# nextpyp/spr_pick

Measured on AMD Instinct MI355X. Metric: train_patches_per_sec, higher is better.
Workload: dtype f32; 1 GPU; BASELINE configs[1]: ssdn --noise_style gaussian --noise_value var, joint mode, 64x64 patches from 4 synthetic 1024x1024 micrographs, batch 32 per GPU, alpha 0.75, tau 0.01, Adam; fp32 MFMA convolutions (Winograd F(2x2,3x3) for the wide 3x3 layers); per_gpu_batch=32, global_batch=32, patch=64, parallelism=single GPU

## Files before the change

include/sprk.h:

```cpp
#ifndef SPRK_H
#define SPRK_H

#include <stddef.h>
#include <stdint.h>

#ifdef __cplusplus
extern "C" {
#endif

#define SPRK_OK 0
#define SPRK_EINVAL (-1)
#define SPRK_EWORKSPACE (-2)
#define SPRK_ELAUNCH (-3)

#define SPRK_ACT_NONE 0
#define SPRK_ACT_LEAKY 1
#define SPRK_ACT_RELU 2

typedef struct sprk_conv_geom {
    int32_t N, C1, C2, Hin, Win, up1;
    int32_t Cout, Hout, Wout;
    int32_t KH, KW, stride, dil, pad_top, pad_left;
    int32_t dtype;
} sprk_conv_geom;

#define SPRK_DT_F32 0
#define SPRK_DT_BF16 1
#define SPRK_DT_F16 2
#define SPRK_DT_MASK 0xff
#define SPRK_DT_FORCE 0x100
#define SPRK_DT_NAIVE 0x200
#define SPRK_DT_PIN 0x400
#define SPRK_DT_X16 0x8000
#define SPRK_DT_Y16 0x10000
#define SPRK_IO2(a, b) ((a) | ((b) << 4))
#define SPRK_IO3(a, b, c) ((a) | ((b) << 4) | ((c) << 8))

typedef struct sprk_conv_epilogue {
    const float *bias, *scale, *shift, *res;
    int32_t res_h, res_w, res_off;
    int32_t act;
    int32_t up2;
} sprk_conv_epilogue;

#define SPRK_ABI_VERSION 430
const char *sprk_last_error(void);
int sprk_version(void);
size_t sprk_struct_bytes(int which);
long sprk_launch_count(void);
long sprk_wino_launch_count(void);
long sprk_mask1x1_launch_count(void);
long sprk_gemm1x1_launch_count(void);
void sprk_gemm1x1_enable(int on);
long sprk_wgrad1x1_launch_count(void);
void sprk_wgrad1x1_enable(int on);
long sprk_conv16_launch_count(void);
long sprk_wgrad16_launch_count(void);

size_t sprk_conv2d_fwd_ws_bytes(const sprk_conv_geom *g);
int sprk_conv2d_fwd(const float *x, const float *x2, const float *w, float *y,
                    const sprk_conv_geom *g, const sprk_conv_epilogue *ep,
                    void *ws, size_t ws_bytes, void *stream);
size_t sprk_conv2d_bwd_data_ws_bytes(const sprk_conv_geom *g);
int sprk_conv2d_bwd_data(const float *gy, const float *w, float *gin, const sprk_conv_geom *g,
                         void *ws, size_t ws_bytes, void *stream);
size_t sprk_head1x1_fwd_ws_bytes(int K0, int N1);
int sprk_head1x1_fwd(const float *f, const float *w1, const float *b1, const float *w2, const float *b2,
                     const float *w3, const float *b3, float *out, int B, int K0, int N1, int N3, long HW, void *ws,
                     size_t ws_bytes, void *stream);

int sprk_head1x1_unrot_fwd(const float *d, const float *w1, const float *b1, const float *w2, const float *b2,
                           const float *w3, const float *b3, float *out, int B, int C, int P, int N3, void *ws,
                           size_t ws_bytes, void *stream);

int sprk_conv2d_bwd_data_masked(const float *gy, const float *w, float *gin, const sprk_conv_geom *g,
                                const float *mask_y, int mask_act, void *ws, size_t ws_bytes, void *stream);
int sprk_conv2d_bwd_data_mask_fused(const sprk_conv_geom *g);
int sprk_conv2d_storage16(const sprk_conv_geom *g, const sprk_conv_epilogue *ep);
size_t sprk_conv2d_bwd_weight_ws_bytes(const sprk_conv_geom *g);
int sprk_conv2d_bwd_weight(const float *x, const float *x2, const float *gy, float *gw,
                           const sprk_conv_geom *g, void *ws, size_t ws_bytes, void *stream);
#define SPRK_VARIANT_INTS 24
#define SPRK_STAGE_NONE (-2)
#define SPRK_STAGE_REFUSED (-1)
#define SPRK_STAGE_DIRECT 0
#define SPRK_STAGE_STEM 1
#define SPRK_STAGE_16BIT 2
#define SPRK_STAGE_WINOGRAD 3
#define SPRK_STAGE_MASK1X1 4
#define SPRK_STAGE_MFMA 5
#define SPRK_STAGE_GEMM1X1 6
#define SPRK_STAGE_WGRAD1X1 7
int sprk_conv2d_variant(int which, const sprk_conv_geom *g, const sprk_conv_epilogue *ep, const void *x, const void *x2,
                        const void *y_or_gy, int32_t *out);
int sprk_conv2d_last_variant(int which, int32_t *out);

#define SPRK_DT_WPREP 0x800
#define SPRK_DT_WPREP_KIND(kind) (((kind) & 7) << 12)
#define SPRK_DT_WPREP_KIND_OF(dtype) (((dtype) >> 12) & 7)
typedef struct sprk_wprep_item {
    const float *w;
    void *dst;
    int32_t kind, blocks;
    int32_t p[12];
} sprk_wprep_item;
int sprk_conv2d_fwd_wprep(const float *w, const sprk_conv_geom *g, const sprk_conv_epilogue *ep, void *ws,
                          size_t ws_bytes, sprk_wprep_item *item);
int sprk_conv2d_bwd_data_wprep(const float *w, const sprk_conv_geom *g, void *ws, size_t ws_bytes, sprk_wprep_item *item);
int sprk_prepare_weights(const sprk_wprep_item *items, int n, void *stream);

size_t sprk_act_bwd_ws_bytes(int N, int C, int HW);
int sprk_act_bwd(const void *gy, const void *y, void *gpre, float *gbias, int act,
                 int N, int C, int H, int W, int up2, long g_image_stride, int io,
                 void *ws, size_t ws_bytes, void *stream);
#define SPRK_RED_NONE 0
#define SPRK_RED_ROWS 1
#define SPRK_RED_COLS 2
#define SPRK_RED_WGRAD 3
typedef struct sprk_reduce_item {
    const float *src;
    float *dst;
    int kind, parts, n, K, Cout, CoutP;
} sprk_reduce_item;
int sprk_conv2d_bwd_weight_partial(const float *x, const float *x2, const float *gy, float *gw,
                                   const sprk_conv_geom *g, void *ws, size_t ws_bytes,
                                   sprk_reduce_item *item, void *stream);
int sprk_act_bwd_partial(const void *gy, const void *y, void *gpre, float *gbias, int act,
                         int N, int C, int H, int W, int up2, long g_image_stride, int io,
                         void *ws, size_t ws_bytes, sprk_reduce_item *item, void *stream);
int sprk_reduce_items(const sprk_reduce_item *items, int n, void *stream);

int sprk_concat_up_bwd(const float *gin, float *ga, float *gb, int N, int C1, int C2, int H, int W,
                       int up1, void *stream);

int sprk_shift_maxpool2_fwd(const void *x, void *y, int NC, int H, int W, int shift, int io, void *stream);
int sprk_shift_maxpool2_bwd(const void *gy, const void *x, void *gx, int NC, int H, int W, int shift, int act,
                            int io, void *stream);
int sprk_rot4_stack_fwd(const float *x, float *y, int B, int C, int P, void *stream);
int sprk_rot4_stack_bwd(const float *gy, float *gx, int B, int C, int P, void *stream);
int sprk_unrot4_shift_concat_fwd(const void *d, void *f, int B, int C, int P, int io, void *stream);
int sprk_unrot4_shift_concat_bwd(const void *gf, void *gd, int B, int C, int P, int io, void *stream);
int sprk_unrot_act_bwd_eligible(int B, int C, int P, int act);
int sprk_conv2d_fwd_unrot_eligible(const sprk_conv_geom *g, const sprk_conv_epilogue *ep);
int sprk_conv2d_fwd_unrot(const float *x, const float *x2, const float *w, float *f, const sprk_conv_geom *g,
                          const sprk_conv_epilogue *ep, void *ws, size_t ws_bytes, void *stream);
// ... 120 lines not shown
```

spr_pick_amd/_lib.py:

```python
import ctypes
import os

_HERE = os.path.dirname(os.path.abspath(__file__))
LIB_PATH = os.environ.get("SPRK_LIB") or os.path.join(_HERE, "libsprk.so")

ACT_NONE, ACT_LEAKY, ACT_RELU = 0, 1, 2
DT_F32, DT_BF16, DT_F16 = 0, 1, 2
DT_NAIVE = 0x200
DT_WPREP = 0x800
DT_X16, DT_Y16 = 0x8000, 0x10000
DT_PIN = 0x400
DT_FORCE = 0x100
DTYPES = {"f32": DT_F32, "fp32": DT_F32, "bf16": DT_BF16, "f16": DT_F16, "fp16": DT_F16,
          "bf16!": DT_BF16 | DT_FORCE, "f16!": DT_F16 | DT_FORCE}

c_f = ctypes.c_void_p
c_i = ctypes.c_int
c_vp = ctypes.c_void_p
c_sz = ctypes.c_size_t


class ConvGeom(ctypes.Structure):
    _fields_ = [(n, ctypes.c_int32) for n in
                ("N", "C1", "C2", "Hin", "Win", "up1", "Cout", "Hout", "Wout",
                 "KH", "KW", "stride", "dil", "pad_top", "pad_left", "dtype")]


class ConvEpilogue(ctypes.Structure):
    _fields_ = [("bias", c_vp), ("scale", c_vp), ("shift", c_vp), ("res", c_vp),
                ("res_h", ctypes.c_int32), ("res_w", ctypes.c_int32), ("res_off", ctypes.c_int32),
                ("act", ctypes.c_int32), ("up2", ctypes.c_int32)]


class AdamItem(ctypes.Structure):
    _fields_ = [("p", c_vp), ("g", c_vp), ("m", c_vp), ("v", c_vp), ("n", ctypes.c_long)]


class ReduceItem(ctypes.Structure):
    _fields_ = [("src", c_vp), ("dst", c_vp), ("kind", ctypes.c_int32), ("parts", ctypes.c_int32), ("n", ctypes.c_int32),
                ("K", ctypes.c_int32), ("Cout", ctypes.c_int32), ("CoutP", ctypes.c_int32)]


class WprepItem(ctypes.Structure):
    _fields_ = [("w", c_vp), ("dst", c_vp), ("kind", ctypes.c_int32), ("blocks", ctypes.c_int32), ("p", ctypes.c_int32 * 12)]


_SIGS = {
    "sprk_last_error": (ctypes.c_char_p, []),
    "sprk_version": (c_i, []),
    "sprk_struct_bytes": (c_sz, [c_i]),
    "sprk_launch_count": (ctypes.c_long, []),
    "sprk_wino_launch_count": (ctypes.c_long, []),
    "sprk_mask1x1_launch_count": (ctypes.c_long, []),
    "sprk_gemm1x1_launch_count": (ctypes.c_long, []),
    "sprk_gemm1x1_enable": (None, [c_i]),
    "sprk_wgrad1x1_launch_count": (ctypes.c_long, []),
    "sprk_wgrad1x1_enable": (None, [c_i]),
    "sprk_conv16_launch_count": (ctypes.c_long, []),
    "sprk_wgrad16_launch_count": (ctypes.c_long, []),
    "sprk_conv2d_fwd_ws_bytes": (c_sz, [ctypes.POINTER(ConvGeom)]),
    "sprk_conv2d_fwd": (c_i, [c_f, c_f, c_f, c_f, ctypes.POINTER(ConvGeom), ctypes.POINTER(ConvEpilogue), c_vp, c_sz, c_vp]),
    "sprk_conv2d_fwd_wprep": (c_i, [c_f, ctypes.POINTER(ConvGeom), ctypes.POINTER(ConvEpilogue), c_vp, c_sz, ctypes.POINTER(WprepItem)]),
    "sprk_conv2d_bwd_data_wprep": (c_i, [c_f, ctypes.POINTER(ConvGeom), c_vp, c_sz, ctypes.POINTER(WprepItem)]),
    "sprk_prepare_weights": (c_i, [ctypes.POINTER(WprepItem), c_i, c_vp]),
    "sprk_head1x1_fwd_ws_bytes": (c_sz, [c_i, c_i]),
    "sprk_head1x1_fwd": (c_i, [c_f, c_f, c_f, c_f, c_f, c_f, c_f, c_f, c_i, c_i, c_i, c_i, ctypes.c_long, c_vp, c_sz, c_vp]),
    "sprk_head1x1_unrot_fwd": (c_i, [c_f, c_f, c_f, c_f, c_f, c_f, c_f, c_f, c_i, c_i, c_i, c_i, c_vp, c_sz, c_vp]),
    "sprk_conv2d_bwd_data_ws_bytes": (c_sz, [ctypes.POINTER(ConvGeom)]),
    "sprk_conv2d_bwd_data": (c_i, [c_f, c_f, c_f, ctypes.POINTER(ConvGeom), c_vp, c_sz, c_vp]),
    "sprk_conv2d_bwd_data_masked": (c_i, [c_f, c_f, c_f, ctypes.POINTER(ConvGeom), c_f, c_i, c_vp, c_sz, c_vp]),
    "sprk_conv2d_bwd_weight_ws_bytes": (c_sz, [ctypes.POINTER(ConvGeom)]),
    "sprk_conv2d_storage16": (c_i, [ctypes.POINTER(ConvGeom), ctypes.POINTER(ConvEpilogue)]),
    "sprk_conv2d_bwd_weight": (c_i, [c_f, c_f, c_f, c_f, ctypes.POINTER(ConvGeom), c_vp, c_sz, c_vp]),
    "sprk_conv2d_bwd_weight_partial": (c_i, [c_f, c_f, c_f, c_f, ctypes.POINTER(ConvGeom), c_vp, c_sz, ctypes.POINTER(ReduceItem), c_vp]),
    "sprk_act_bwd_partial": (c_i, [c_f, c_f, c_f, c_f, c_i, c_i, c_i, c_i, c_i, c_i, ctypes.c_long, c_i, c_vp, c_sz, ctypes.POINTER(ReduceItem), c_vp]),
    "sprk_reduce_items": (c_i, [ctypes.POINTER(ReduceItem), c_i, c_vp]),
    "sprk_act_bwd_ws_bytes": (c_sz, [c_i, c_i, c_i]),
    "sprk_act_bwd": (c_i, [c_f, c_f, c_f, c_f, c_i, c_i, c_i, c_i, c_i, c_i, ctypes.c_long, c_i, c_vp, c_sz, c_vp]),
    "sprk_concat_up_bwd": (c_i, [c_f, c_f, c_f, c_i, c_i, c_i, c_i, c_i, c_i, c_vp]),
    "sprk_shift_maxpool2_fwd": (c_i, [c_f, c_f, c_i, c_i, c_i, c_i, c_i, c_vp]),
    "sprk_shift_maxpool2_bwd": (c_i, [c_f, c_f, c_f, c_i, c_i, c_i, c_i, c_i, c_i, c_vp]),
    "sprk_rot4_stack_fwd": (c_i, [c_f, c_f, c_i, c_i, c_i, c_vp]),
    "sprk_rot4_stack_bwd": (c_i, [c_f, c_f, c_i, c_i, c_i, c_vp]),
    "sprk_unrot4_shift_concat_fwd": (c_i, [c_f, c_f, c_i, c_i, c_i, c_i, c_vp]),
    "sprk_unrot4_shift_concat_bwd": (c_i, [c_f, c_f, c_i, c_i, c_i, c_i, c_vp]),
    "sprk_unrot_act_bwd_eligible": (c_i, [c_i, c_i, c_i, c_i]),
    "sprk_conv2d_fwd_unrot_eligible": (c_i, [ctypes.POINTER(ConvGeom), ctypes.POINTER(ConvEpilogue)]),
    "sprk_conv2d_bwd_data_mask_fused": (c_i, [ctypes.POINTER(ConvGeom)]),
    "sprk_conv2d_variant": (c_i, [c_i, ctypes.POINTER(ConvGeom), ctypes.POINTER(ConvEpilogue), c_vp, c_vp, c_vp,
                                  ctypes.POINTER(ctypes.c_int32)]),
    "sprk_conv2d_last_variant": (c_i, [c_i, ctypes.POINTER(ctypes.c_int32)]),
    "sprk_conv2d_fwd_unrot": (c_i, [c_f, c_f, c_f, c_f, ctypes.POINTER(ConvGeom), ctypes.POINTER(ConvEpilogue), c_vp, c_sz, c_vp]),
    "sprk_unrot_act_bwd": (c_i, [c_f, c_f, c_f, c_f, c_i, c_i, c_i, c_i, c_vp, c_sz, ctypes.POINTER(ReduceItem), c_vp]),
    "sprk_bn_ws_bytes": (c_sz, [c_i, c_i, c_i, c_i]),
    "sprk_bn_train_fwd": (c_i, [c_f, c_f, c_f, c_f, c_f, c_f, c_f, c_f, c_i, c_i, c_i, c_i, ctypes.c_float, ctypes.c_float, c_i, c_vp, c_sz, c_vp]),
    "sprk_bn_eval_fwd": (c_i, [c_f, c_f, c_f, c_f, c_f, c_f, c_i, c_i, c_i, ctypes.c_float, c_i, c_vp]),
    "sprk_bn_train_bwd": (c_i, [c_f, c_f, c_f, c_f, c_f, c_f, c_f, c_f, c_f, c_i, c_i, c_i, c_i, c_i, c_vp, c_sz, c_vp]),
    "sprk_crop_add_fwd": (c_i, [c_f, c_f, c_f, ctypes.c_long, c_i, c_i, c_i, c_i, c_i, c_i, c_vp]),
    "sprk_crop_embed_bwd": (c_i, [c_f, c_f, ctypes.c_long, c_i, c_i, c_i, c_i, c_i, c_i, c_vp]),
    "sprk_noise_std_fwd": (c_i, [c_f, c_f, c_f, c_i, c_i, c_vp]),
    "sprk_noise_std_bwd": (c_i, [c_f, c_f, c_f, c_i, c_i, c_vp]),
    "sprk_joint_loss_fwd": (c_i, [c_f, c_f, c_f, c_f, c_f, c_f, c_i, c_i, c_i, c_i, ctypes.c_float, ctypes.c_float, c_vp]),
    "sprk_joint_loss_bwd": (c_i, [c_f, c_f, c_f, c_f, c_f, c_f, c_f, c_i, c_i, c_i, c_i, ctypes.c_float, ctypes.c_float, c_vp]),
    "sprk_reparam_fwd": (c_i, [c_f, c_f, c_f, c_i, c_i, c_vp]),
    "sprk_reparam_bwd": (c_i, [c_f, c_f, c_f, c_f, c_i, c_i, c_vp]),
    "sprk_adam_multi": (c_i, [c_vp, c_vp, c_i, c_i, c_f, c_f, c_f, ctypes.c_float, ctypes.c_float, ctypes.c_float, c_vp]),
    "sprk_adam_multi_skip": (c_i, [c_vp, c_vp, c_i, c_i, c_f, c_f, c_f, ctypes.c_float, ctypes.c_float, ctypes.c_float, c_vp, c_vp]),
    "sprk_unscale_check": (c_i, [c_f, ctypes.c_long, c_f, c_vp, c_vp]),
    "sprk_loss_scale_update": (c_i, [c_f, c_f, c_vp, c_vp, c_vp, c_vp, ctypes.c_float, ctypes.c_float, c_i, c_vp]),
    "sprk_pu_loss": (c_i, [c_f, c_f, c_f, c_i, ctypes.c_float, c_f, c_f, c_vp]),
# ... 70 lines not shown
```

spr_pick_amd/csrc/conv.hip:

```cpp
#include "common.h"
#include "conv16.h"
#include "gemm1x1.h"
#include "mask1x1.h"
#include "wgrad16.h"
#include "wgrad1x1.h"
#include "wino.h"
#include "wprep_dev.h"

#include <cstdlib>

#include "conv_dev.h"
#include "io_dev.h"


namespace {

inline bool naive_of(const sprk_conv_geom *g) { return (g->dtype & SPRK_DT_NAIVE) != 0; }

constexpr int kZeroFloats = 256;
__device__ __attribute__((aligned(64))) float g_zero_block[kZeroFloats];

__device__ __forceinline__ void stage_planes(float *dst, const float *base, long imgStride, long cs, int nch, int N,
                                             int Hin, int Win, int Ws, int up, int vec, const float *zeros,
                                             const PlaneGeom &g, int n0, int iy0, int ixa, int lw, int lane) {
    const int imgElems = g.inRows * g.pitch;
    const int planeElems = g.NI * imgElems;
    const int per = vec ? 256 : 64;
    const int nGroups = (planeElems + per - 1) / per;
    const int nw = g.nw;
    const int gstart = g.deal ? 0 : lw, gstep = g.deal ? 1 : nw, cstep = g.deal ? nw : 1;
    for (int gi = gstart; gi < nGroups; gi += gstep) {
        const int e = vec ? gi * 256 + lane * 4 : gi * 64 + lane;
        const int il = fast_div(e, g.invImg);
        const int rem = e - il * imgElems;
        const int r = fast_div(rem, g.invPitch);
        const int j = rem - r * g.pitch;
        const int n = n0 + il, iy = iy0 + r, ix = ixa + j;
        const bool inb = e < planeElems;
        const bool ok = inb && n < N && (unsigned)iy < (unsigned)Hin && (unsigned)ix < (unsigned)Win;
        const int cl0 = g.deal ? (lw + nw - (gi % nw)) % nw : 0;
        const float *p = base + (long)n * imgStride + (up ? (long)(iy >> 1) * Ws + (ix >> 1) : (long)iy * Ws + ix) +
                         (long)cl0 * cs;
        long step = (long)cstep * cs;
        if (!ok) {
            p = zeros + lane * 4;
            step = 0;
        }
        float *d = dst + gi * per + cl0 * g.cplane;
        for (int cl = cl0; cl < nch; cl += cstep) {
            if (inb) {
                if (vec)
                    dma16(p, d);
                else
                    dma4(p, d);
            }
            p += step;
            d += cstep * g.cplane;
        }
// ... 1622 lines not shown
    return rc == sprk::kWprepDescribed ? (int)SPRK_OK : rc;
}

int sprk_conv2d_bwd_data(const float *gy, const float *w, float *gin, const sprk_conv_geom *g, void *ws,
                         size_t ws_bytes, void *stream) {
    return sprk_conv2d_bwd_data_masked(gy, w, gin, g, nullptr, SPRK_ACT_NONE, ws, ws_bytes, stream);
}

int sprk_conv2d_bwd_data_masked(const float *gy, const float *w, float *gin, const sprk_conv_geom *g,
                                const float *mask_y, int mask_act, void *ws, size_t ws_bytes, void *stream) {
    sprk::WprepScope scope(nullptr, g ? g->dtype : 0);
    return scope.verify(conv_dispatch(true, gy, nullptr, w, gin, g, nullptr, mask_y, mask_act, ws, ws_bytes, stream));
}

int sprk_conv2d_bwd_data_mask_fused(const sprk_conv_geom *g) {
    if (!g || check_geom(g) != SPRK_OK || naive_of(g) || g->stride != 1 || g->up1) return 0;
    const sprk::Corr c(*g);
    if (c.dt() != SPRK_DT_F32 && sprk::conv16_eligible(c)) return 0;
    if (c.dtype & (SPRK_DT_X16 | SPRK_DT_Y16)) return 0;
    if (sprk::wino_eligible(c)) return 1;
    FwdPlan p;
    return (plan_fwd(c, &p) && mask1x1_takes(g, c, p)) ? 1 : 0;
}

int sprk_conv2d_bwd_data_wprep(const float *w, const sprk_conv_geom *g, void *ws, size_t ws_bytes, sprk_wprep_item *item) {
    SPRK_REQUIRE(item && w && ws, "conv2d_bwd_data_wprep: null argument");
    *item = sprk_wprep_item{};
    sprk::WprepScope scope(item, 0);
    const int rc = conv_dispatch(true, (const float *)ws, nullptr, w, (float *)ws, g, nullptr, nullptr, SPRK_ACT_NONE, ws,
                                 ws_bytes, nullptr);
    return rc == sprk::kWprepDescribed ? (int)SPRK_OK : rc;
}

static size_t wgrad_ws_bytes(const sprk_conv_geom &g) {
    size_t need = sprk::wgrad16_ws_bytes(g);
    WgPlan p;
    if (sprk::wino_wgrad_eligible(g)) need = std::max(need, sprk::wino_wgrad_ws_bytes(g));
    if (plan_wgrad(&g, &p)) need = std::max(need, p.wsBytes);
    return need;
}

size_t sprk_conv2d_bwd_weight_ws_bytes(const sprk_conv_geom *g) { return g ? wgrad_ws_bytes(*g) : 0; }

static bool wgrad1x1_takes(const sprk_conv_geom *g, const WgPlan &p, const WgVariant &v) {
    const int W = g->Wout, H = g->Hout;
    const bool rows64 = W % 64 == 0 || ((W == 4 || W == 8 || W == 16 || W == 32) && H % (64 / W) == 0 && H * W >= 64);
    return sprk::g_wgrad1x1_on.load(std::memory_order_relaxed) && (g->dtype & SPRK_DT_MASK) == SPRK_DT_F32 &&
           !(g->dtype & (SPRK_DT_X16 | SPRK_DT_Y16)) && !naive_of(g) && g->KH == 1 && g->KW == 1 && g->stride == 1 &&
           g->pad_top == 0 && g->pad_left == 0 && g->C2 == 0 && !g->up1 && g->Hin == g->Hout && g->Win == g->Wout &&
           v.stage == SPRK_STAGE_MFMA && p.xrow && v.MODE == 1 && p.IT == 3 && p.NT == 6 && p.CKW <= sprk::kWgrad1x1Rows &&
           rows64 && (long)sprk::kWgrad1x1Rows * H * W * 4 < (1L << 31);
}

static WgVariant wg_route(const sprk_conv_geom *g, const void *x, const void *x2, const void *gy, WgPlan *p) {
    WgVariant v{};
    const bool naive = naive_of(g);
    if (!naive && sprk::wgrad16_ws_bytes(*g)) {
        v.stage = SPRK_STAGE_16BIT;
        sprk::wgrad16_variant(*g, v.rec16);
    } else if (g->dtype & (SPRK_DT_X16 | SPRK_DT_Y16)) {
        v.stage = SPRK_STAGE_REFUSED;
    } else if (!naive && sprk::wino_wgrad_eligible(*g)) {
        v.stage = SPRK_STAGE_WINOGRAD;
        v.wino = sprk::wino_wgrad_variant(*g);
    } else if (naive || !plan_wgrad(g, p)) {
        v.stage = SPRK_STAGE_DIRECT;
    } else {
        bool refused;
        v = wg_variant(g, *p, x, x2, gy, &refused);
        v.stage = refused ? SPRK_STAGE_REFUSED : SPRK_STAGE_MFMA;
        if (wgrad1x1_takes(g, *p, v)) v.stage = SPRK_STAGE_WGRAD1X1;
    }
    return v;
}

static int wgrad_dispatch(const float *x, const float *x2, const float *gy, float *gw, const sprk_conv_geom *g, void *ws,
                          size_t ws_bytes, sprk_reduce_item *item, void *stream) {
    const char *who = "conv2d_bwd_weight";
    if (item) *item = sprk_reduce_item{nullptr, nullptr, SPRK_RED_NONE, 0, 0, 0, 0, 0};
    if (int rc = check_geom(g)) return rc;
    SPRK_REQUIRE(x && gy && gw, "conv2d_bwd_weight: null tensor");
    SPRK_REQUIRE(g->C2 == 0 || x2, "conv2d_bwd_weight: C2 > 0 but x2 is null");
    hipStream_t s = (hipStream_t)stream;

    WgPlan p;
    const WgVariant v = wg_route(g, x, x2, gy, &p);
    t_last_wg = v;

    if (v.stage == SPRK_STAGE_16BIT) {
        if (int rc = sprk::check_ws(who, ws, ws_bytes, sprk::wgrad16_ws_bytes(*g))) return rc;
        return sprk::wgrad16_run(*g, x, x2, gy, gw, ws, item, s);
    }
    if (int rc = check_storage32(who, g->dtype)) return rc;

    if (v.stage == SPRK_STAGE_WINOGRAD) {
        if (int rc = sprk::check_ws(who, ws, ws_bytes, sprk::wino_wgrad_ws_bytes(*g))) return rc;
        return sprk::wino_wgrad(*g, v.wino, x, x2, gy, gw, ws, item, s);
    }

    if (v.stage == SPRK_STAGE_DIRECT) {
        DirectArgs a{x, x2, nullptr, gy, gw, *g, sprk::kNoEpilogue};
        hipLaunchKernelGGL(conv_bwd_weight_direct_kernel, dim3(g->Cout * (g->C1 + g->C2)), dim3(256), 0, s, a);
        return sprk::check_launch("conv_bwd_weight_direct");
    }
    if (int rc = sprk::check_ws(who, ws, ws_bytes, p.wsBytes)) return rc;
    SPRK_REQUIRE(v.stage != SPRK_STAGE_REFUSED,
                 "conv2d_bwd_weight: 1x1 row staging needs 16-byte aligned x / gy and < 2^28-element tiles");
    float *wsf = (float *)ws;
    if (v.stage == SPRK_STAGE_WGRAD1X1) {
        const sprk::Wgrad1x1Call c{x, gy, wsf + kZeroFloats, g->N, g->C1, g->Cout, p.CoutP, g->Hout * g->Wout,
                                   p.nTiles, p.tilesPerGroup, p.groups, p.CKW, p.nChunks, p.nblkN};
        sprk::prof_begin(1, sprk::conv_flops(*g), s);
        if (int rc = sprk::wgrad1x1_run(c, s)) return rc;
        sprk::prof_end(1, s);
        if (int rc2 = sprk::check_launch("wgrad1x1")) return rc2;
    } else {
        WgArgs a;
        if (int rc = wgrad_args(g, p, v, x, x2, gy, wsf, a)) return rc;
        sprk::prof_begin(1, sprk::conv_flops(*g), s);
        if (int rc = launch_wg(a, p, v, s)) return rc;
        sprk::prof_end(1, s);
        if (int rc2 = sprk::check_launch("conv_wgrad_mfma")) return rc2;
    }
    const int K = (g->C1 + g->C2) * g->KH * g->KW;
    const sprk_reduce_item it{wsf + kZeroFloats, gw, SPRK_RED_WGRAD, p.groups, 0, K, g->Cout, p.CoutP};
    return sprk::finish_or_defer(it, item, s);
}

static void variant_out(const FwdVariant &v, int32_t *out) {
    if (v.stage == SPRK_STAGE_16BIT) {
        out[0] = v.stage;
        for (int i = 1; i < SPRK_VARIANT_INTS; ++i) out[i] = v.rec16[i];
        return;
    }
    if (v.stage == SPRK_STAGE_WINOGRAD) {
        const sprk::WinoVariant &w = v.wino;
        const int f[] = {v.stage, w.NT, w.SQ, w.UNROT, w.groups, w.lastCh, w.nc1, w.nch, w.r1, w.r2, w.pairs, w.sw, w.gridX,
                         w.ntiles, w.tpwMin, w.tpwMax, w.xcd, w.tilesX, w.tilesY, w.padT, w.padL, w.mode};
        static_assert(sizeof(f) / sizeof(f[0]) <= SPRK_VARIANT_INTS, "the record fits");
        for (int i = 0; i < SPRK_VARIANT_INTS; ++i) out[i] = i < (int)(sizeof(f) / sizeof(f[0])) ? f[i] : 0;
        return;
    }
    const int f[] = {v.stage, v.MT, v.NT, v.RB, v.XTAB, v.small, v.stages, v.ragged_k, v.latency, v.vec1, v.vec2, v.vec4,
                     v.colOff, v.up1, v.c2, v.taps, v.CK, v.nChunks, v.blocks};
    for (int i = 0; i < SPRK_VARIANT_INTS; ++i) out[i] = i < (int)(sizeof(f) / sizeof(f[0])) ? f[i] : 0;
}
static void variant_out(const WgVariant &v, int32_t *out) {
    if (v.stage == SPRK_STAGE_16BIT) {
        out[0] = v.stage;
        for (int i = 1; i < SPRK_VARIANT_INTS; ++i) out[i] = v.rec16[i];
        return;
    }
    if (v.stage == SPRK_STAGE_WINOGRAD) {
        const sprk::WinoWgVariant &w = v.wino;
        int f[SPRK_VARIANT_INTS] = {v.stage, w.launches};
        for (int i = 0; i < w.launches; ++i) f[2 + 3 * i] = w.l[i].MT, f[3 + 3 * i] = w.l[i].ch, f[4 + 3 * i] = w.l[i].parts;
        int srcMask = 0;
        for (int i = 0; i < w.launches; ++i) srcMask |= w.l[i].src << i;
        const int t[] = {w.regionsX, w.regionsY, w.cx, w.cy, w.padT, w.padL, w.Cout, w.xcdMask, srcMask};
        static_assert(14 + sizeof(t) / sizeof(t[0]) <= SPRK_VARIANT_INTS, "the record fits");
        for (int i = 0; i < (int)(sizeof(t) / sizeof(t[0])); ++i) f[14 + i] = t[i];
        for (int i = 0; i < SPRK_VARIANT_INTS; ++i) out[i] = f[i];
        return;
    }
    const int f[] = {v.stage, v.IT, v.NT, v.WJ, v.MODE, v.xrow, v.xtab, v.g4, v.vec1, v.vec2, v.chunks, v.groups, v.up1, v.c2,
                     v.tiles};
    for (int i = 0; i < SPRK_VARIANT_INTS; ++i) out[i] = i < (int)(sizeof(f) / sizeof(f[0])) ? f[i] : 0;
}
// ... 128 lines not shown
```

spr_pick_amd/csrc/core.hip:

```cpp
#include "common.h"
#include "wprep_dev.h"
#include "conv16.h"
#include "gemm1x1.h"
#include "wgrad1x1.h"
#include "wgrad16.h"

#include <mutex>
#include <tuple>
#include <vector>

namespace sprk {

static thread_local char t_error[512] = "";
std::atomic<long> g_launches{0}, g_wino_launches{0}, g_mask1x1_launches{0};

void set_error(const char *fmt, ...) {
    va_list ap;
    va_start(ap, fmt);
    vsnprintf(t_error, sizeof(t_error), fmt, ap);
    va_end(ap);
}

constexpr int kMaxDev = 64;
int num_cus() {
    static std::atomic<int> cus[kMaxDev];
    int dev = 0;
    if (hipGetDevice(&dev) != hipSuccess || dev < 0 || dev >= kMaxDev) return 256;
    int v = cus[dev].load(std::memory_order_relaxed);
    if (v == 0) {
        if (hipDeviceGetAttribute(&v, hipDeviceAttributeMultiprocessorCount, dev) != hipSuccess || v <= 0) v = 256;
        cus[dev].store(v, std::memory_order_relaxed);
    }
    return v;
}

int lds_optin(const void *kernel, size_t bytes, const char *what) {
    if (bytes <= 64 * 1024) return SPRK_OK;
    static std::mutex mu;
    static std::vector<std::tuple<int, const void *, size_t>> done;
    int dev = 0;
    (void)hipGetDevice(&dev);
    std::lock_guard<std::mutex> lk(mu);
    for (auto &d : done)
        if (std::get<0>(d) == dev && std::get<1>(d) == kernel && std::get<2>(d) >= bytes) return SPRK_OK;
    if (hipFuncSetAttribute(kernel, hipFuncAttributeMaxDynamicSharedMemorySize, (int)bytes) != hipSuccess) {
        set_error("%s: cannot reserve %zu bytes of LDS", what, bytes);
        return SPRK_ELAUNCH;
    }
    done.emplace_back(dev, kernel, bytes);
    return SPRK_OK;
}

struct ProfRec {
    hipEvent_t a, b;
    int kclass;
    double flops, bytes;
};
// ... 187 lines not shown
    set_error("prepared weights: the workspace holds a transform of another kind than this call's kernel path reads");
    return SPRK_EINVAL;
}
bool wprep_describing() { return t_wprep_describe != nullptr; }
int wprep_site(const sprk_wprep_item &it, hipStream_t s) {
    if (t_wprep_describe) {
        *t_wprep_describe = it;
        return kWprepDescribed;
    }
    if (t_wprep_skip) {
        t_wprep_seen = it.kind;
        if (t_wprep_expect && it.kind != t_wprep_expect) {
            set_error("prepared weights: the workspace holds a transform of another kind than this call's kernel path reads");
            return SPRK_EINVAL;
        }
        return SPRK_OK;
    }
    return wprep_launch(&it, 1, s);
}

}

extern "C" {

int sprk_prepare_weights(const sprk_wprep_item *items, int n, void *stream) {
    SPRK_REQUIRE(n >= 0 && (n == 0 || items), "prepare_weights: bad arguments");
    return sprk::wprep_launch(items, n, (hipStream_t)stream);
}

int sprk_reduce_items(const sprk_reduce_item *items, int n, void *stream) {
    SPRK_REQUIRE(n >= 0 && (n == 0 || items), "reduce_items: bad arguments");
    return sprk::reduce_items(items, n, (hipStream_t)stream);
}

const char *sprk_last_error(void) { return sprk::t_error; }
int sprk_version(void) { return SPRK_ABI_VERSION; }
size_t sprk_struct_bytes(int which) {
    switch (which) {
    case 0: return sizeof(sprk_conv_geom);
    case 1: return sizeof(sprk_conv_epilogue);
    case 2: return sizeof(sprk_reduce_item);
    case 3: return sizeof(sprk_adam_item);
    case 4: return sizeof(sprk_wprep_item);
    default: return 0;
    }
}
long sprk_launch_count(void) { return sprk::g_launches.load(); }
long sprk_wino_launch_count(void) { return sprk::g_wino_launches.load(); }
long sprk_mask1x1_launch_count(void) { return sprk::g_mask1x1_launches.load(); }
long sprk_gemm1x1_launch_count(void) { return sprk::g_gemm1x1_launches.load(); }
void sprk_gemm1x1_enable(int on) { sprk::g_gemm1x1_on.store(on ? 1 : 0); }
long sprk_wgrad1x1_launch_count(void) { return sprk::g_wgrad1x1_launches.load(); }
void sprk_wgrad1x1_enable(int on) { sprk::g_wgrad1x1_on.store(on ? 1 : 0); }
long sprk_conv16_launch_count(void) { return sprk::conv16_launches() + sprk::wgrad16_launches(); }
long sprk_wgrad16_launch_count(void) { return sprk::wgrad16_launches(); }

void sprk_prof_enable(int on) {
    std::lock_guard<std::mutex> lk(sprk::g_prof_mu);
    sprk::g_prof_mask = on;
}

int sprk_prof_collect(int kclass, long *launches, double *ms, double *flops) {
    return sprk_prof_collect_bytes(kclass, launches, ms, flops, nullptr);
}

int sprk_prof_collect_bytes(int kclass, long *launches, double *ms, double *flops, double *bytes) {
    std::lock_guard<std::mutex> lk(sprk::g_prof_mu);
    long n = 0;
    double t = 0.0, f = 0.0, by = 0.0;
    std::vector<sprk::ProfRec> keep;
    for (auto &r : sprk::g_recs) {
        if (r.kclass != kclass) {
            keep.push_back(r);
            continue;
        }
        float dt = 0.f;
        if (hipEventSynchronize(r.b) == hipSuccess && hipEventElapsedTime(&dt, r.a, r.b) == hipSuccess) {
            ++n;
            t += dt;
            f += r.flops;
            by += r.bytes;
        }
        sprk::g_pool.push_back({r.a, r.b});
    }
    sprk::g_recs.swap(keep);
    if (launches) *launches = n;
    if (ms) *ms = t;
    if (flops) *flops = f;
    if (bytes) *bytes = by;
    return SPRK_OK;
}

}
```

Measured before the change: 2034 patches/s.

## Add specialized MFMA weight-gradient kernel for 3x3 fp32 convolutions

Adds a dedicated wgrad3x3 kernel for stride-1 3x3 fp32 weight-gradient convolutions that the generic MFMA path would otherwise handle. It stages 48-channel input chunks and output-gradient tiles into double-buffered LDS with buffer DMA, then feeds 16x16x4 MFMAs from shared LDS images across the 27 k-tiles of a chunk. It is enabled by default and gated on a narrow set of plan parameters. The aim is more data reuse and overlap of loads with compute in the wide 3x3 layers' weight gradients, at the cost of large LDS use and a hand-scheduled pipeline that is more fragile. Scratch benchmarking scripts are included.

```diff
diff --git a/include/sprk.h b/include/sprk.h
--- a/include/sprk.h
+++ b/include/sprk.h
@@ -54,6 +54,8 @@
 void sprk_gemm1x1_enable(int on);
 long sprk_wgrad1x1_launch_count(void);
 void sprk_wgrad1x1_enable(int on);
+long sprk_wgrad3x3_launch_count(void);
+void sprk_wgrad3x3_enable(int on);
 long sprk_conv16_launch_count(void);
 long sprk_wgrad16_launch_count(void);
 
@@ -91,6 +93,7 @@
 #define SPRK_STAGE_MFMA 5
 #define SPRK_STAGE_GEMM1X1 6
 #define SPRK_STAGE_WGRAD1X1 7
+#define SPRK_STAGE_WGRAD3X3 8
 int sprk_conv2d_variant(int which, const sprk_conv_geom *g, const sprk_conv_epilogue *ep, const void *x, const void *x2,
                         const void *y_or_gy, int32_t *out);
 int sprk_conv2d_last_variant(int which, int32_t *out);
diff --git a/scratch/wgrad3x3_bench.py b/scratch/wgrad3x3_bench.py
--- /dev/null
+++ b/scratch/wgrad3x3_bench.py
@@ -0,0 +1,110 @@
+import ctypes
+import json
+import statistics
+import sys
+
+import torch
+
+from spr_pick_amd import _lib, ops
+
+GEOM = ("N", "C1", "C2", "Hin", "Win", "up1", "Cout", "Hout", "Wout", "KH", "KW", "stride", "dil", "pad_top", "pad_left", "dtype")
+
+
+def last_record(L):
+    out = (ctypes.c_int32 * 24)()
+    L.sprk_conv2d_last_variant(2, out)
+    return list(out)
+
+
+def do_list(path):
+    sys.path.insert(0, ".")
+    from bench import make_cfg
+    from spr_pick_amd import Denoiser, graph_step, synthetic
+    L = _lib.lib()
+    calls = []
+
+    def wrap(name, igeom):
+        real = getattr(L, name)
+
+        def f(*a):
+            rc = real(*a)
+            g = a[igeom]._obj
+            calls.append({"geom": [int(getattr(g, k)) for k in GEOM],
+                          "aligned16": [(ctypes.cast(p, ctypes.c_void_p).value or 0) % 16 == 0 for p in a[:3]],
+                          "record": last_record(L)})
+            return rc
+        setattr(L, name, f)
+
+    wrap("sprk_conv2d_bwd_weight", 4)
+    wrap("sprk_conv2d_bwd_weight_partial", 4)
+    dev = torch.device("cuda:0")
+    torch.manual_seed(0)
+    den = Denoiser(make_cfg(), device=dev, mode="joint")
+    den.train()
+    st = graph_step.GraphedTrainStep(den, 32, 64, 0.75, 0.01, graph=False)
+    inp, tgt = synthetic.patch_batches(1, 32, [synthetic.micrograph(i) for i in range(2)], seed=100, device=dev)[0]
+    st(inp, tgt, eager=True)
+    torch.cuda.synchronize()
+    calls.clear()
+    st(inp, tgt, eager=True)
+    torch.cuda.synchronize()
+    json.dump({"geom_fields": GEOM, "calls": calls}, open(path, "w"), indent=0)
+    for i, c in enumerate(calls):
+        g, r = dict(zip(GEOM, c["geom"])), c["record"]
+        print("%3d N%4d C%3d+%3d %3dx%-3d up%d -> %3d k%d s%d d%d pad %d,%d  stage %d IT %d NT %d WJ %d MODE %d chunks %d groups %d c2 %d tiles %d" % (
+            i, g["N"], g["C1"], g["C2"], g["Hin"], g["Win"], g["up1"], g["Cout"], g["KH"], g["stride"], g["dil"], g["pad_top"],
+            g["pad_left"], r[0], r[1], r[2], r[3], r[4], r[10], r[11], r[13], r[14]))
+
+
+def do_run(path, reps, only):
+    L, S, dev = _lib.lib(), torch.ops.sprk, torch.device("cuda:0")
+    have = "sprk_wgrad3x3_enable" in _lib.EXPORTS
+    calls = [c for c in json.load(open(path))["calls"]
+             if c["record"][0] == 5 and c["record"][4] == 2 and c["geom"][9] == 3 and c["geom"][10] == 3]
+    seen, uniq = set(), []
+    for c in calls:
+        if tuple(c["geom"]) not in seen:
+            seen.add(tuple(c["geom"]))
+            uniq.append(c)
+    gen = torch.Generator().manual_seed(1)
+    for i, c in enumerate(uniq):
+        if only and i not in only:
+            continue
+        g = dict(zip(GEOM, c["geom"]))
+        x = torch.randn(g["N"], g["C1"], g["Hin"], g["Win"], generator=gen).to(dev)
+        x2 = torch.randn(g["N"], g["C2"], g["Hin"], g["Win"], generator=gen).to(dev) if g["C2"] else None
+        gy = torch.randn(g["N"], g["Cout"], g["Hout"], g["Wout"], generator=gen).to(dev)
+        gw = torch.empty(g["Cout"], g["C1"] + g["C2"], 3, 3, device=dev)
+        geom = [g[k] for k in GEOM]
+        res = {}
+        for on in ((0, 1) if have else (None,)):
+            if on is not None:
+                L.sprk_wgrad3x3_enable(on)
+            ts = []
+            for _ in range(reps):
+                a, b = torch.cuda.Event(enable_timing=True), torch.cuda.Event(enable_timing=True)
+                a.record()
+                S.conv2d_bwd_weight(x, x2, gy, geom, gw, False)
+                b.record()
+                torch.cuda.synchronize()
+                ts.append(a.elapsed_time(b) * 1e3)
+            res[on] = gw.clone()
+            r = last_record(L)
+            print("CALL %d switch %s N %d C %d+%d %dx%d -> %d pad %d,%d  stage %d IT %d NT %d chunks %d groups %d tiles %d  "
+                  "median %.1f us min %.1f (reduction included; %.1f TF)" % (
+                      i, on, g["N"], g["C1"], g["C2"], g["Hin"], g["Win"], g["Cout"], g["pad_top"], g["pad_left"], r[0], r[1],
+                      r[2], r[10], r[11], r[14], statistics.median(ts), min(ts),
+                      18.0 * g["N"] * g["Hout"] * g["Wout"] * (g["C1"] + g["C2"]) * g["Cout"] / statistics.median(ts) * 1e-6),
+                  flush=True)
+        if have:
+            print("    on == off: %s" % torch.equal(res[0].view(torch.int32), res[1].view(torch.int32)), flush=True)
+        del x, x2, gy, gw, res
+        torch.cuda.empty_cache()
+
+
+if __name__ == "__main__":
+    if sys.argv[1] == "list":
+        do_list(sys.argv[2])
+    else:
+        do_run(sys.argv[2], int(sys.argv[3]) if len(sys.argv) > 3 else 5,
+               [int(t) for t in sys.argv[4].split(",")] if len(sys.argv) > 4 else [])
diff --git a/scratch/wgrad3x3_step_trace.py b/scratch/wgrad3x3_step_trace.py
--- /dev/null
+++ b/scratch/wgrad3x3_step_trace.py
@@ -0,0 +1,39 @@
+import csv
+import glob
+import os
+import re
+import sys
+
+d, steps = sys.argv[1], int(sys.argv[2]) if len(sys.argv) > 2 else 8
+pat = re.compile("conv_wgrad_mfma_kernel|wgrad1x1_kernel|wgrad3x3_kernel")
+DRIFT = (("gemm1x1_kernel<2", None), ("wgrad1x1_kernel", None), ("wino_conv_kernel<6, 0, 1", None),
+         ("unrot_act_bwd64_kernel", None), ("wino_wgrad_kernel<3", "131072"))
+
+
+def short(n):
+    n = re.sub(r"\(anonymous namespace\)::", "", n)
+    n = re.sub(r"^void ", "", n)
+    return n.split("(")[0][:48]
+
+
+def med(v):
+    v = sorted(v)
+    return v[len(v) // 2]
+
+
+for f in sorted(glob.glob(os.path.join(d, "**", "*kernel_trace.csv"), recursive=True)):
+    rows = sorted((int(r["Start_Timestamp"]), short(r["Kernel_Name"]), r.get("Grid_Size_X", ""),
+                   (int(r["End_Timestamp"]) - int(r["Start_Timestamp"])) / 1e3) for r in csv.DictReader(open(f)))
+    main = [r for r in rows if pat.search(r[1])]
+    gs = [r[2] for r in main]
+    period = next(m for m in range(1, len(gs) // 3) if gs[-m:] == gs[-2 * m:-m] == gs[-3 * m:-2 * m] and len(set(gs[-m:])) > 1)
+    use = min(steps, len(gs) // period - 1)
+    tail = main[-use * period:]
+    print("%s: %d launches, period %d, %d steps used" % (os.path.basename(f), len(main), period, use))
+    for p in range(period):
+        v = [tail[s * period + p][3] for s in range(use)]
+        print("POS %2d %-44s grid %7s  median %.1f us  min %.1f" % (p, tail[p][1], tail[p][2], med(v), min(v)))
+    for name, grid in DRIFT:
+        v = [r[3] for r in rows if name in r[1] and (grid is None or r[2] == grid)]
+        if v:
+            print("DRIFT %-44s grid %7s  n %d  median %.1f us" % (name, grid or "any", len(v), med(v)))
diff --git a/scratch/wgrad3x3_summary.py b/scratch/wgrad3x3_summary.py
--- /dev/null
+++ b/scratch/wgrad3x3_summary.py
@@ -0,0 +1,43 @@
+import csv
+import glob
+import os
+import re
+import sys
+from collections import defaultdict
+
+d, reps = sys.argv[1], int(sys.argv[2])
+pat = re.compile("conv_wgrad_mfma_kernel|wgrad3x3_kernel")
+
+
+def short(n):
+    n = re.sub(r"\(anonymous namespace\)::", "", n)
+    n = re.sub(r"^void ", "", n)
+    return n.split("(")[0][:48]
+
+
+def runs(rows):
+    rows.sort(key=lambda r: r[0])
+    return [rows[i:i + reps] for i in range(0, len(rows), reps)]
+
+
+for f in sorted(glob.glob(os.path.join(d, "**", "*kernel_trace.csv"), recursive=True)):
+    rows = [(int(r["Start_Timestamp"]), short(r["Kernel_Name"]), r.get("Grid_Size_X", ""), r.get("Workgroup_Size_X", ""),
+             (int(r["End_Timestamp"]) - int(r["Start_Timestamp"])) / 1e3)
+            for r in csv.DictReader(open(f)) if pat.search(r["Kernel_Name"])]
+    for i, run in enumerate(runs(rows)):
+        v = sorted(r[4] for r in run)
+        print("TRACE run %2d %-44s grid %7s wg %s  n %d  median %.1f us  min %.1f" % (
+            i, run[0][1], run[0][2], run[0][3], len(v), v[len(v) // 2], v[0]))
+for f in sorted(glob.glob(os.path.join(d, "**", "*counter_collection.csv"), recursive=True)):
+    disp = defaultdict(dict)
+    meta = {}
+    for r in csv.DictReader(open(f)):
+        if pat.search(r["Kernel_Name"]):
+            k = int(r["Dispatch_Id"])
+            disp[k][r["Counter_Name"]] = disp[k].get(r["Counter_Name"], 0.0) + float(r["Counter_Value"])
+            meta[k] = (short(r["Kernel_Name"]), r.get("Grid_Size", ""), r.get("VGPR_Count", ""), r.get("Accum_VGPR_Count", ""),
+                       r.get("LDS_Block_Size", ""), r.get("Scratch_Size", ""))
+    for i, run in enumerate(runs([(k, v) for k, v in disp.items()])):
+        print("PMC run %2d %-44s grid %s vgpr %s agpr %s lds %s scratch %s" % ((i,) + meta[run[0][0]]))
+        for c in sorted(run[0][1]):
+            print("      %-28s mean %.6g  (n %d)" % (c, sum(r[1].get(c, 0.0) for r in run) / len(run), len(run)))
diff --git a/spr_pick_amd/_lib.py b/spr_pick_amd/_lib.py
--- a/spr_pick_amd/_lib.py
+++ b/spr_pick_amd/_lib.py
@@ -56,6 +56,8 @@
     "sprk_gemm1x1_enable": (None, [c_i]),
     "sprk_wgrad1x1_launch_count": (ctypes.c_long, []),
     "sprk_wgrad1x1_enable": (None, [c_i]),
+    "sprk_wgrad3x3_launch_count": (ctypes.c_long, []),
+    "sprk_wgrad3x3_enable": (None, [c_i]),
     "sprk_conv16_launch_count": (ctypes.c_long, []),
     "sprk_wgrad16_launch_count": (ctypes.c_long, []),
     "sprk_conv2d_fwd_ws_bytes": (c_sz, [ctypes.POINTER(ConvGeom)]),
diff --git a/spr_pick_amd/csrc/conv.hip b/spr_pick_amd/csrc/conv.hip
--- a/spr_pick_amd/csrc/conv.hip
+++ b/spr_pick_amd/csrc/conv.hip
@@ -4,6 +4,7 @@
 #include "mask1x1.h"
 #include "wgrad16.h"
 #include "wgrad1x1.h"
+#include "wgrad3x3.h"
 #include "wino.h"
 #include "wprep_dev.h"
 
@@ -1732,6 +1733,15 @@
            rows64 && (long)sprk::kWgrad1x1Rows * H * W * 4 < (1L << 31);
 }
 
+static bool wgrad3x3_takes(const sprk_conv_geom *g, const WgPlan &p, const WgVariant &v) {
+    return sprk::g_wgrad3x3_on.load(std::memory_order_relaxed) && (g->dtype & SPRK_DT_MASK) == SPRK_DT_F32 &&
+           !(g->dtype & (SPRK_DT_X16 | SPRK_DT_Y16)) && !naive_of(g) && g->KH == 3 && g->KW == 3 && g->stride == 1 &&
+           g->dil == 1 && !g->up1 && g->Hin == g->Hout && g->Win == g->Wout && g->pad_top >= 0 && g->pad_top <= 2 &&
+           g->pad_left >= 0 && g->pad_left <= 2 && v.stage == SPRK_STAGE_MFMA && v.MODE == 2 && p.IT == 7 &&
+           (p.NT == 3 || p.NT == 6) && p.CKW == sprk::kWgrad3x3Chunk && g->C1 % p.CKW == 0 && g->C2 % p.CKW == 0 &&
+           sprk::wgrad3x3_plane(g->Hout, g->Wout) && (1 << p.lgTC) == g->Wout && (64 >> p.lgTC) == (1 << p.lgTR);
+}
+
 static WgVariant wg_route(const sprk_conv_geom *g, const void *x, const void *x2, const void *gy, WgPlan *p) {
     WgVariant v{};
     const bool naive = naive_of(g);
@@ -1750,6 +1760,7 @@
         v = wg_variant(g, *p, x, x2, gy, &refused);
         v.stage = refused ? SPRK_STAGE_REFUSED : SPRK_STAGE_MFMA;
         if (wgrad1x1_takes(g, *p, v)) v.stage = SPRK_STAGE_WGRAD1X1;
+        else if (wgrad3x3_takes(g, *p, v)) v.stage = SPRK_STAGE_WGRAD3X3;
     }
     return v;
 }
@@ -1794,6 +1805,13 @@
         if (int rc = sprk::wgrad1x1_run(c, s)) return rc;
         sprk::prof_end(1, s);
         if (int rc2 = sprk::check_launch("wgrad1x1")) return rc2;
+    } else if (v.stage == SPRK_STAGE_WGRAD3X3) {
+        const sprk::Wgrad3x3Call c{x, x2, gy, wsf + kZeroFloats, g->N, g->C1, g->C2, g->Cout, p.CoutP, g->Hout, g->Wout,
+                                   g->pad_top, g->pad_left, p.NT, p.nTiles, p.tilesPerGroup, p.groups, p.nChunks, p.nblkN};
+        sprk::prof_begin(1, sprk::conv_flops(*g), s);
+        if (int rc = sprk::wgrad3x3_run(c, s)) return rc;
+        sprk::prof_end(1, s);
+        if (int rc2 = sprk::check_launch("wgrad3x3")) return rc2;
     } else {
         WgArgs a;
         if (int rc = wgrad_args(g, p, v, x, x2, gy, wsf, a)) return rc;
diff --git a/spr_pick_amd/csrc/core.hip b/spr_pick_amd/csrc/core.hip
--- a/spr_pick_amd/csrc/core.hip
+++ b/spr_pick_amd/csrc/core.hip
@@ -3,6 +3,7 @@
 #include "conv16.h"
 #include "gemm1x1.h"
 #include "wgrad1x1.h"
+#include "wgrad3x3.h"
 #include "wgrad16.h"
 
 #include <mutex>
@@ -296,6 +297,8 @@
 void sprk_gemm1x1_enable(int on) { sprk::g_gemm1x1_on.store(on ? 1 : 0); }
 long sprk_wgrad1x1_launch_count(void) { return sprk::g_wgrad1x1_launches.load(); }
 void sprk_wgrad1x1_enable(int on) { sprk::g_wgrad1x1_on.store(on ? 1 : 0); }
+long sprk_wgrad3x3_launch_count(void) { return sprk::g_wgrad3x3_launches.load(); }
+void sprk_wgrad3x3_enable(int on) { sprk::g_wgrad3x3_on.store(on ? 1 : 0); }
 long sprk_conv16_launch_count(void) { return sprk::conv16_launches() + sprk::wgrad16_launches(); }
 long sprk_wgrad16_launch_count(void) { return sprk::wgrad16_launches(); }
 
diff --git a/spr_pick_amd/csrc/wgrad3x3.h b/spr_pick_amd/csrc/wgrad3x3.h
--- /dev/null
+++ b/spr_pick_amd/csrc/wgrad3x3.h
@@ -0,0 +1,25 @@
+#pragma once
+#include "common.h"
+
+namespace sprk {
+
+struct Wgrad3x3Call {
+    const float *x, *x2, *gy;
+    float *partial;
+    int N, C1, C2, Cout, CoutP;
+    int H, W, padT, padL;
+    int NT;
+    int nTiles, tilesPerGroup, groups;
+    int nChunks, nblkN;
+};
+
+constexpr int kWgrad3x3Chunk = 48;
+
+inline bool wgrad3x3_plane(int H, int W) { return (W == 16 || W == 32 || W == 64) && H >= 64 / W && H % (64 / W) == 0; }
+
+int wgrad3x3_run(const Wgrad3x3Call &c, hipStream_t s);
+
+extern std::atomic<long> g_wgrad3x3_launches;
+extern std::atomic<int> g_wgrad3x3_on;
+
+}
diff --git a/spr_pick_amd/csrc/wgrad3x3.hip b/spr_pick_amd/csrc/wgrad3x3.hip
--- /dev/null
+++ b/spr_pick_amd/csrc/wgrad3x3.hip
@@ -0,0 +1,238 @@
+#include "wgrad3x3.h"
+
+#include <type_traits>
+
+#include "conv_dev.h"
+
+namespace {
+
+constexpr int kCK = sprk::kWgrad3x3Chunk;
+constexpr int kCS = 288;
+constexpr int kXFloats = kCK * kCS + 32;
+constexpr int NW = 8;
+constexpr int kXDma = kCK / NW;
+static_assert(kCS % 32 == 0 && kCS >= 256 + 27 + 1 && kXFloats % 4 == 0, "x image");
+
+struct W3Args {
+    const float *x, *x2, *gy;
+    float *partial;
+    int C1, C2, Cout, CoutP, H, padT, padL;
+    int tilesPerImg, nTiles, tilesPerGroup;
+};
+
+typedef const __attribute__((address_space(3))) f32x4 *lds_c4p;
+
+__device__ __forceinline__ int zoff(int c) { return (c & 3) + 8 * ((c >> 2) & 3); }
+
+template <int KT, int LGW>
+__global__ __launch_bounds__(64 * NW) void wgrad3x3_kernel(const W3Args a) {
+    constexpr int NT = KT == 4 ? 3 : 6;
+    constexpr int NTW = 3;
+    constexpr int KS = KT == 4 ? 8 : 4;
+    constexpr int kCols = NT * 16;
+    constexpr int W = 1 << LGW, TR = 64 / W, Q = W / 4 + 2, P = 4 * Q, U = (TR + 2) * Q;
+    constexpr int kGDma = (NT * 4 + NW - 1) / NW;
+    constexpr int kStageFloats = kXFloats + kCols * 64;
+    constexpr int kStageBytes = kStageFloats * 4;
+    static_assert(U <= 64 && KT * KS + 3 >= 27, "one wave DMA per channel; every k-tile has an owner");
+    extern __shared__ __attribute__((aligned(16))) float smem[];
+    const int tid = threadIdx.x, lane = tid & 63;
+    const int wave = __builtin_amdgcn_readfirstlane(tid >> 6);
+    const int l15 = lane & 15, lq = lane >> 4;
+    const int k0 = KT == 4 ? wave : (wave & 3);
+    const int g0 = KT == 4 ? 0 : (wave >> 2) * NTW;
+    const int nk = (27 - k0 + KS - 1) / KS;
+    const int c0 = blockIdx.y * kCK;
+    const int second = c0 >= a.C1 ? 1 : 0;
+    const float *src = second ? a.x2 : a.x;
+    const int Cs = second ? a.C2 : a.C1, cs0 = c0 - (second ? a.C1 : 0);
+    const int co0 = blockIdx.z * kCols;
+    const int plane = a.H * W;
+    const int t_begin = blockIdx.x * a.tilesPerGroup;
+    const int nt = min(a.nTiles, t_begin + a.tilesPerGroup) - t_begin;
+
+    const int rl = lane / Q, ql = lane - rl * Q;
+    const int xcol = (lane < U && ql >= 1 && ql <= W / 4) ? (rl * W + 4 * ql - 4) * 4 : kXZero;
+    int gv[kGDma], ggi[kGDma];
+#pragma unroll
+    for (int i = 0; i < kGDma; ++i) {
+        int gi = wave + NW * i;
+        if (gi >= NT * 4) gi -= NT * 4;
+        const int r = 4 * gi + lq;
+        ggi[i] = gi;
+        gv[i] = (co0 + r < a.Cout) ? (r * plane + ((l15 ^ (r & 15)) << 2)) * 4 : kXZero;
+    }
+
+    const int n0 = __builtin_amdgcn_readfirstlane(t_begin / a.tilesPerImg);
+    int ty = __builtin_amdgcn_readfirstlane(t_begin - n0 * a.tilesPerImg);
+    long xo = ((long)n0 * Cs + cs0) * plane + (long)(ty * TR - a.padT) * W;
+    long go = ((long)n0 * a.Cout + co0) * plane + ty * 64;
+    int left = __builtin_amdgcn_readfirstlane(nt - 1);
+    const int xwrap = (Cs - 1) * plane, gwrap = (a.Cout - 1) * plane;
+    auto advance = [&]() {
+        const int more = left > 0 ? 1 : 0;
+        const int wrap = (ty + 1 == a.tilesPerImg ? 1 : 0) & more;
+        left -= more;
+        ty = (ty + more) & (wrap - 1);
+        xo += more * 64 + wrap * xwrap;
+        go += more * 64 + wrap * gwrap;
+    };
+    const int chanStep = NW * plane * 4;
+    auto issue = [&](int b) {
+        const rsrc_t xr = make_rsrc(src + xo), gr = make_rsrc(a.gy + go);
+        const int iy = ty * TR - a.padT + rl;
+        const int xv = (unsigned)iy < (unsigned)a.H ? xcol : kXZero;
+        float *xs = smem + b * kStageFloats;
+        float *gs = xs + kXFloats;
+#pragma unroll
+        for (int i = 0; i < kXDma; ++i) {
+            const int c = wave + NW * i;
+            bdma16(xr, xv, wave * (plane * 4) + i * chanStep, xs + c * kCS + zoff(c));
+        }
+#pragma unroll
+        for (int i = 0; i < kGDma; ++i) bdma16(gr, gv[i], 0, gs + ggi[i] * 256);
+    };
+
+    int ab[KT], boff[4];
+    {
+        const int lbase = lds_addr(smem) + (l15 * kCS + zoff(l15)) * 4 + 16 * lq;
+#pragma unroll
+        for (int t = 0; t < KT; ++t) {
+            const int kt = min(k0 + KS * t, 26);
+            const int tap = kt / 3, cb = kt - 3 * tap, ky = tap / 3, kx = tap - 3 * ky;
+            ab[t] = lbase + (cb * 16 * kCS + ky * P + kx - a.padL + 4) * 4;
+        }
+#pragma unroll
+        for (int j = 0; j < 4; ++j)
+            boff[j] = lds_addr(smem) + (kXFloats + (g0 * 16 + l15) * 64) * 4 + (((4 * j) ^ lq ^ l15) << 4);
+    }
+    f32x4 acc[KT][NTW];
+#pragma unroll
+    for (int t = 0; t < KT; ++t)
+#pragma unroll
+        for (int n = 0; n < NTW; ++n) acc[t][n] = f32x4{0.f, 0.f, 0.f, 0.f};
+
+    auto tiles = [&](auto nkc) {
+        constexpr int NK = decltype(nkc)::value;
+        float a0[NK], a1[NK];
+        f32x4 b0[NTW], b1[NTW];
+        auto ldA = [&](float (&av)[NK], int so, int ks) {
+            const int j = ks >> 2, s = ks & 3;
+#pragma unroll
+            for (int t = 0; t < NK; ++t) av[t] = lds_f(ab[t] + so)[((16 * j) >> LGW) * P + ((16 * j) & (W - 1)) + s];
+        };
+        auto ldB = [&](f32x4 (&bv)[NTW], int so, int j) {
+#pragma unroll
+            for (int n = 0; n < NTW; ++n) bv[n] = *(lds_c4p)(__SIZE_TYPE__)(unsigned)(boff[j] + so + n * (16 * 256));
+        };
+        auto mm = [&](const float (&av)[NK], const f32x4 (&bv)[NTW], int s) {
+#pragma unroll
+            for (int t = 0; t < NK; ++t)
+#pragma unroll
+                for (int n = 0; n < NTW; ++n)
+                    acc[t][n] = __builtin_amdgcn_mfma_f32_16x16x4f32(av[t], bv[n][s], acc[t][n], 0, 0, 0);
+        };
+        issue(0);
+        advance();
+        issue(1);
+        advance();
+        asm volatile("s_waitcnt vmcnt(0)" ::: "memory");
+        lds_only_barrier();
+        ldA(a0, 0, 0);
+        ldB(b0, 0, 0);
+        for (int i = 0; i < nt; ++i) {
+            const int so = (i & 1) * kStageBytes, son = kStageBytes - so;
+#pragma unroll
+            for (int j = 0; j < 4; ++j) {
+                if (j + 1 < 4) {
+                    if (j & 1) ldB(b0, so, j + 1); else ldB(b1, so, j + 1);
+                }
+#pragma unroll
+                for (int s = 0; s < 4; ++s) {
+                    const int ks = 4 * j + s;
+                    if (ks + 1 < 16) {
+                        if (ks & 1) ldA(a0, so, ks + 1); else ldA(a1, so, ks + 1);
+                    }
+                    if (ks == 15) {
+                        ldA(a0, son, 0);
+                        ldB(b0, son, 0);
+                    }
+                    if (ks & 1) {
+                        if (j & 1) mm(a1, b1, s); else mm(a1, b0, s);
+                    } else {
+                        if (j & 1) mm(a0, b1, s); else mm(a0, b0, s);
+                    }
+                    if (ks == 14) {
+                        asm volatile("s_waitcnt vmcnt(0)" ::: "memory");
+                        lds_only_barrier();
+                        issue(i & 1);
+                        advance();
+                    }
+                }
+            }
+        }
+        asm volatile("s_waitcnt vmcnt(0)" ::: "memory");
+    };
+    if (nt > 0) {
+        if (nk == KT)
+            tiles(std::integral_constant<int, KT>{});
+        else
+            tiles(std::integral_constant<int, KT - 1>{});
+    }
+
+    float *dst = a.partial + (long)blockIdx.x * (a.C1 + a.C2) * 9 * a.CoutP;
+#pragma unroll
+    for (int t = 0; t < KT; ++t) {
+        const int kt = k0 + KS * t;
+        if (kt >= 27) continue;
+        const int tap = kt / 3, cb = kt - 3 * tap;
+#pragma unroll
+        for (int j = 0; j < 4; ++j) {
+            const int c = c0 + cb * 16 + lq * 4 + j;
+#pragma unroll
+            for (int n = 0; n < NTW; ++n) dst[((long)c * 9 + tap) * a.CoutP + co0 + (g0 + n) * 16 + l15] = acc[t][n][j];
+        }
+    }
+}
+
+template <int KT, int LGW>
+int launch3x3(const W3Args &a, dim3 grid, hipStream_t s) {
+    constexpr size_t lds = 2 * (size_t)(kXFloats + (KT == 4 ? 3 : 6) * 16 * 64) * 4;
+    if (int rc = sprk::lds_optin(wgrad3x3_kernel<KT, LGW>, lds, "wgrad3x3")) return rc;
+    hipLaunchKernelGGL((wgrad3x3_kernel<KT, LGW>), grid, dim3(64 * NW), lds, s, a);
+    return SPRK_OK;
+}
+
+template <int KT>
+int launch3x3_w(const W3Args &a, int W, dim3 grid, hipStream_t s) {
+    return W == 16 ? launch3x3<KT, 4>(a, grid, s) : W == 32 ? launch3x3<KT, 5>(a, grid, s) : launch3x3<KT, 6>(a, grid, s);
+}
+
+}
+
+namespace sprk {
+
+std::atomic<long> g_wgrad3x3_launches{0};
+std::atomic<int> g_wgrad3x3_on{1};
+
+int wgrad3x3_run(const Wgrad3x3Call &c, hipStream_t s) {
+    const int Cin = c.C1 + c.C2;
+    const long plane = (long)c.H * c.W;
+    SPRK_REQUIRE(wgrad3x3_plane(c.H, c.W) && (c.NT == 3 || c.NT == 6) && c.C1 > 0 && c.C1 % kCK == 0 && c.C2 % kCK == 0 &&
+                     (c.C2 == 0 || c.x2) && c.nChunks == Cin / kCK && c.nblkN == cdiv(c.Cout, c.NT * 16) &&
+                     c.CoutP == c.nblkN * c.NT * 16 && c.padT >= 0 && c.padT <= 2 && c.padL >= 0 && c.padL <= 2 &&
+                     (long)std::max(c.C1, c.C2) * plane < (1L << 28) && (long)c.Cout * plane < (1L << 28) &&
+                     c.nTiles == (long)c.N * (plane / 64) && c.tilesPerGroup >= 1 &&
+                     c.groups == cdiv(c.nTiles, c.tilesPerGroup),
+                 "wgrad3x3: call outside the kernel's limits");
+    W3Args a{};
+    a.x = c.x; a.x2 = c.x2; a.gy = c.gy; a.partial = c.partial;
+    a.C1 = c.C1; a.C2 = c.C2; a.Cout = c.Cout; a.CoutP = c.CoutP; a.H = c.H; a.padT = c.padT; a.padL = c.padL;
+    a.tilesPerImg = (int)(plane / 64); a.nTiles = c.nTiles; a.tilesPerGroup = c.tilesPerGroup;
+    const dim3 grid(c.groups, c.nChunks, c.nblkN);
+    if (int rc = c.NT == 3 ? launch3x3_w<4>(a, c.W, grid, s) : launch3x3_w<7>(a, c.W, grid, s)) return rc;
+    g_wgrad3x3_launches.fetch_add(1, std::memory_order_relaxed);
+    return SPRK_OK;
+}
+
+}
```

Result: faster. 2056 patches/s, median of 6 (+1.1%).
